# Aedelon/MASt3R-SLAM

Measured on AMD Instinct MI355X. Metric: keyframe-pairs/sec (512x512 two-view infer+match+GN), higher is better.
Workload: dtype fp16

## Files before the change

### mast3r-slam_amd/csrc/conv_tail.hip

```cpp
#include "gemm_common.h"

using namespace m3gemm;

namespace {

constexpr int kThreads = 512;
constexpr int TH = 16, TW = 32;
constexpr int HH = TH + 2, HW = TW + 2;
constexpr int kHaloPix = HH * HW;
constexpr int kHaloBytes = kHaloPix * 128;
constexpr int kWStage = 128 * 128;
constexpr int PH = 11, PW = 19;
constexpr int kPatchBytes = (PH * PW * 128 + 1023) / 1024 * 1024;
constexpr int kLdsBytes = kHaloBytes + 2 * kWStage + kPatchBytes;

struct TailArgs {
    const bf16_t *X;
    const bf16_t *Wc;
    const float *bias;
    const bf16_t *W4;
    const float *b4;
    float *pts, *conf;
    bf16_t *Y;
    const bf16_t *R;
    int cout, relu_in;
    const bf16_t *zero16;
    int B, H, W, IH, IW;
    const bf16_t *Wc2, *W42;
    const float *bias2, *b42;
};

enum { EP_PLAIN = 0 , EP_TAIL = 1 , EP_RELU = 2 ,
       EP_ADD = 3  };

template <int DT, bool UPS, int CIN, int EP>
__global__ void __launch_bounds__(kThreads, 2)
k_conv_tail(const TailArgs ain) {
    constexpr bool TAIL = EP == EP_TAIL;
    static_assert(CIN % 64 == 0 && (TAIL ? CIN == 128 : true), "64-channel steps; the fused tail is the 128-channel head.2");
    constexpr int NQ = CIN / 64;
    TailArgs a = ain;
    if (blockIdx.y == 1) {
        a.Wc = ain.Wc2; a.W4 = ain.W42; a.bias = ain.bias2; a.b4 = ain.b42;
        a.X = ain.X + (size_t)ain.B * ain.IH * ain.IW * CIN;
        if (TAIL) {
            a.pts = ain.pts + (size_t)ain.B * ain.H * ain.W * 3;
            a.conf = ain.conf + (size_t)ain.B * ain.H * ain.W;
        } else {
            a.Y = ain.Y + (size_t)ain.B * ain.H * ain.W * ain.cout;
            if (EP == EP_ADD) a.R = ain.R + (size_t)ain.B * ain.H * ain.W * ain.cout;
        }
    }
    if (!TAIL) {
        const int z = blockIdx.z;
        a.Wc += (size_t)z * 128 * 9 * CIN;
        if (a.bias) a.bias += z * 128;
        a.Y += z * 128;
        if (EP == EP_ADD) a.R += z * 128;
    }
    extern __shared__ __attribute__((aligned(16))) unsigned char lds[];
    unsigned char *halo = lds, *wst = lds + kHaloBytes, *patch = lds + kHaloBytes + 2 * kWStage;
    const int tid = threadIdx.x, lane = tid & 63, wave = tid >> 6;
    const int wp = wave >> 1, wc = wave & 1;
    const int tiles_x = (a.W + TW - 1) / TW, tiles_y = a.H / TH;
    const int nwg = tiles_x * tiles_y * a.B;
    const int bid = xcd_remap(blockIdx.x, nwg);
    const int b = bid / (tiles_x * tiles_y), trem = bid - b * tiles_x * tiles_y;
    const int ty = trem / tiles_x, tx = trem - ty * tiles_x;
    const int oy0 = ty * TH, ox0 = tx * TW;
    const bf16_t *img = a.X + (size_t)b * a.IH * a.IW * CIN;

    auto stage_w = [&](int tap, int half, int buf) {
        unsigned char *base = wst + buf * kWStage;
#pragma unroll
        for (int i = 0; i < 2; ++i) {
            const int slot = i * kThreads + tid;
            const int row = slot >> 3, cp = slot & 7;
            const int c = half * 8 + (cp ^ ((row >> 1) & 7));
            glds16(a.Wc + ((size_t)row * 9 + tap) * CIN + c * 8, base + i * (kThreads * 16) + wave * 1024);
        }
    };
    const float sy = UPS && a.H > 1 ? (float)(a.IH - 1) / (float)(a.H - 1) : 0.f;
    const float sx = UPS && a.W > 1 ? (float)(a.IW - 1) / (float)(a.W - 1) : 0.f;
    const int py0 = (int)((float)max(oy0 - 1, 0) * sy), px0 = (int)((float)max(ox0 - 1, 0) * sx);
    auto stage_patch = [&](int half) {
        for (int wi = wave; wi < (PH * PW * 8 + 63) / 64; wi += kThreads / 64) {
            int slot = wi * 64 + lane;
            slot = slot < PH * PW * 8 ? slot : PH * PW * 8 - 1;
            const int pp = slot >> 3, c = slot & 7;
            const int y = min(py0 + pp / PW, a.IH - 1), x = min(px0 + pp % PW, a.IW - 1);
            glds16(img + ((size_t)y * a.IW + x) * CIN + (half * 8 + c) * 8, patch + wi * 1024);
        }
    };
    auto stage_halo_direct = [&](int half) {
        for (int wi = wave; wi < (kHaloPix * 8 + 63) / 64; wi += kThreads / 64) {
            int slot = wi * 64 + lane;
            const bool live = slot < kHaloPix * 8;
            slot = live ? slot : kHaloPix * 8 - 1;
            const int pix = slot >> 3, cp = slot & 7;
            const int hy = pix / HW, hx = pix - hy * HW;
            const int iy = oy0 + hy - 1, ix = ox0 + hx - 1;
            const int c = half * 8 + (cp ^ ((hx >> 1) & 7));
            const bool in = iy >= 0 && iy < a.H && ix >= 0 && ix < a.W;
            const void *src = in ? (const void *)(img + ((size_t)iy * a.IW + ix) * CIN + c * 8) : (const void *)a.zero16;
            if (wi * 64 + 64 <= kHaloPix * 8) glds16(src, halo + wi * 1024);
            else if (live) *reinterpret_cast<uint4 *>(halo + (size_t)slot * 16) = *reinterpret_cast<const uint4 *>(src);
        }
    };
    auto blend_halo = [&]() {
        for (int slot = tid; slot < kHaloPix * 8; slot += kThreads) {
            const int pix = slot >> 3, cp = slot & 7;
            const int hy = pix / HW, hx = pix - hy * HW;
            const int iy = oy0 + hy - 1, ix = ox0 + hx - 1;
            const int c = cp ^ ((hx >> 1) & 7);
            uint4 o = make_uint4(0u, 0u, 0u, 0u);
            if (iy >= 0 && iy < a.H && ix >= 0 && ix < a.W) {
                const float fy = iy * sy, fx = ix * sx;
                int y0 = (int)fy, x0 = (int)fx;
                y0 = min(y0, a.IH - 1); x0 = min(x0, a.IW - 1);
                const int y1 = min(y0 + 1, a.IH - 1), x1 = min(x0 + 1, a.IW - 1);
                const float wy = fy - (float)y0, wx = fx - (float)x0;
                const unsigned char *p = patch + c * 16;
                union U { uint4 q; unsigned w[4]; } q00, q01, q10, q11, r;
                q00.q = *reinterpret_cast<const uint4 *>(p + ((y0 - py0) * PW + (x0 - px0)) * 128);
                q01.q = *reinterpret_cast<const uint4 *>(p + ((y0 - py0) * PW + (x1 - px0)) * 128);
                q10.q = *reinterpret_cast<const uint4 *>(p + ((y1 - py0) * PW + (x0 - px0)) * 128);
                q11.q = *reinterpret_cast<const uint4 *>(p + ((y1 - py0) * PW + (x1 - px0)) * 128);
#pragma unroll
                for (int k = 0; k < 4; ++k) {
                    const float tl = lo16<DT>(q00.w[k]) * (1.f - wx) + lo16<DT>(q01.w[k]) * wx;
                    const float bl = lo16<DT>(q10.w[k]) * (1.f - wx) + lo16<DT>(q11.w[k]) * wx;
                    const float th = hi16<DT>(q00.w[k]) * (1.f - wx) + hi16<DT>(q01.w[k]) * wx;
                    const float bh = hi16<DT>(q10.w[k]) * (1.f - wx) + hi16<DT>(q11.w[k]) * wx;
                    r.w[k] = pack16<DT>(tl * (1.f - wy) + bl * wy, th * (1.f - wy) + bh * wy);
                }
                o = r.q;
            }
            *reinterpret_cast<uint4 *>(halo + (size_t)slot * 16) = o;
        }
    };

    f32x4 acc[8][4];
#pragma unroll
    for (int i = 0; i < 8; ++i)
#pragma unroll
        for (int j = 0; j < 4; ++j) acc[i][j] = f32x4{0.f, 0.f, 0.f, 0.f};
    const int frow = lane & 15, fch = lane >> 4;
    int w_off[4];
#pragma unroll
    for (int j = 0; j < 4; ++j) {
        const int r = wc * 64 + j * 16 + frow;
        w_off[j] = r * 128 + ((fch ^ ((r >> 1) & 7)) << 4);
    }

    const int group = wave >> 2;
    bf16x8 af[8], wf[4];
    const int pix_of_row = (int)((0x3D9F2A40E6C851B7ULL >> (4 * frow)) & 15);
    auto col_offset = [&](int hx) { return hx * 128 + ((fch ^ ((hx >> 1) & 7)) << 4); };
    auto read_frags = [&](int g, int tap, int ks) {
        const int ky = tap / 3, kx = tap - ky * 3;
        const unsigned char *wsrc = wst + (g & 1) * kWStage;
        const int flip = ks << 6;
        const int c0 = col_offset(pix_of_row + kx) ^ flip;
        const int c1 = col_offset(16 + pix_of_row + kx) ^ flip;
        const unsigned char *rowp = halo + (wp * 4 + ky) * (HW * 128);
#pragma unroll
        for (int j = 0; j < 4; ++j) wf[j] = *reinterpret_cast<const bf16x8 *>(wsrc + (w_off[j] ^ flip));
#pragma unroll
        for (int i = 0; i < 8; ++i)
            af[i] = *reinterpret_cast<const bf16x8 *>(rowp + (i >> 1) * (HW * 128) + ((i & 1) ? c1 : c0));
        if (!TAIL && a.relu_in) {
#pragma unroll
            for (int i = 0; i < 8; ++i) af[i] = relu_frag(af[i]);
        }
    };
    auto mfma_all = [&]() {
        __builtin_amdgcn_s_setprio(1);
#pragma unroll
        for (int i = 0; i < 8; ++i)
#pragma unroll
            for (int j = 0; j < 4; ++j) acc[i][j] = mfma16<DT>(wf[j], af[i], acc[i][j]);
        __builtin_amdgcn_s_setprio(0);
    };
    auto phase_end = [&]() {
        __builtin_amdgcn_sched_barrier(0);
        __builtin_amdgcn_s_barrier();
        __builtin_amdgcn_sched_barrier(0);
    };
    auto phase_end_wait = [&]() {
        __builtin_amdgcn_sched_barrier(0);
        asm volatile("s_waitcnt vmcnt(0)" ::: "memory");
        __builtin_amdgcn_s_barrier();
        __builtin_amdgcn_sched_barrier(0);
    };
    auto prefetch_w = [&](int g) { if (g + 1 < 9 * NQ) stage_w((g + 1) % 9, (g + 1) / 9, (g + 1) & 1); };
    auto run_half = [&](int half) {
        if (group == 0) {
#pragma unroll 1
            for (int tap = 0; tap < 9; ++tap) {
                const int g = half * 9 + tap;
                read_frags(g, tap, 0);
                prefetch_w(g);
                asm volatile("s_waitcnt lgkmcnt(0)" ::: "memory");
                phase_end();
                mfma_all();
                phase_end();
                read_frags(g, tap, 1);
                asm volatile("s_waitcnt lgkmcnt(0)" ::: "memory");
                phase_end();
                mfma_all();
                phase_end_wait();
            }
            phase_end();
        } else {
#pragma unroll 1
            for (int tap = 0; tap < 9; ++tap) {
                const int g = half * 9 + tap;
                if (tap > 0) mfma_all();
                phase_end();
                read_frags(g, tap, 0);
                prefetch_w(g);
                asm volatile("s_waitcnt lgkmcnt(0)" ::: "memory");
                phase_end();
                mfma_all();
                phase_end();
                read_frags(g, tap, 1);
                asm volatile("s_waitcnt lgkmcnt(0)" ::: "memory");
                phase_end_wait();
            }
            mfma_all();
            phase_end();
        }
    };

    stage_w(0, 0, 0);
    if (UPS) stage_patch(0); else stage_halo_direct(0);
    asm volatile("s_waitcnt vmcnt(0)" ::: "memory");
    lds_barrier();
#pragma unroll 1
    for (int q = 0; q < NQ; ++q) {
        if (UPS) {
            blend_halo();
            lds_barrier();
            if (q + 1 < NQ) stage_patch(q + 1);
        } else if (q > 0) {
            stage_halo_direct(q);
            asm volatile("s_waitcnt vmcnt(0)" ::: "memory");
            lds_barrier();
        }
        run_half(q);
    }

    if constexpr (EP == EP_ADD) {
        const int r = lane & 15, gq = lane >> 4;
        constexpr int RS = 272;
        unsigned char *wl = halo + wave * (32 * RS);
        float4 bj[4];
#pragma unroll
        for (int j = 0; j < 4; ++j)
            bj[j] = a.bias ? *reinterpret_cast<const float4 *>(a.bias + wc * 64 + j * 16 + gq * 4) : make_float4(0.f, 0.f, 0.f, 0.f);
        auto pix = [&](int pass, int rl, int &oy, int &ox) {
            const int i = pass * 2 + (rl >> 4);
            oy = oy0 + wp * 4 + (i >> 1);
            ox = ox0 + (i & 1) * 16 + (int)((0x3D9F2A40E6C851B7ULL >> (4 * (rl & 15))) & 15);
        };
        uint4 q[2][4];
        auto load_resid = [&](int pass, uint4 (&dst)[4]) {
#pragma unroll
            for (int it = 0; it < 4; ++it) {
                const int c = it * 64 + lane, rl = c >> 3, ch = c & 7;
                int oy, ox;
                pix(pass, rl, oy, ox);
                ox = ox < a.W ? ox : a.W - 1;
                dst[it] = *reinterpret_cast<const uint4 *>(a.R + (((size_t)b * a.H + oy) * a.W + ox) * a.cout + wc * 64 + ch * 8);
            }
        };
        load_resid(0, q[0]);
#pragma unroll
        for (int pass = 0; pass < 4; ++pass) {
            if (pass + 1 < 4) load_resid(pass + 1, q[(pass + 1) & 1]);
#pragma unroll
            for (int ii = 0; ii < 2; ++ii)
#pragma unroll
                for (int j = 0; j < 4; ++j) {
                    const f32x4 v = acc[pass * 2 + ii][j];
                    *reinterpret_cast<float4 *>(wl + (ii * 16 + r) * RS + ((j * 4 + gq) << 4)) =
                        make_float4(v[0] + bj[j].x, v[1] + bj[j].y, v[2] + bj[j].z, v[3] + bj[j].w);
                }
            asm volatile("s_waitcnt lgkmcnt(0)" ::: "memory");
#pragma unroll
            for (int it = 0; it < 4; ++it) {
                const int c = it * 64 + lane, rl = c >> 3, ch = c & 7;
                const float4 f0 = *reinterpret_cast<const float4 *>(wl + rl * RS + ch * 32);
                const float4 f1 = *reinterpret_cast<const float4 *>(wl + rl * RS + ch * 32 + 16);
                const uint4 u = q[pass & 1][it];
                uint4 o;
                o.x = pack16<DT>(f0.x + lo16<DT>(u.x), f0.y + hi16<DT>(u.x));
                o.y = pack16<DT>(f0.z + lo16<DT>(u.y), f0.w + hi16<DT>(u.y));
                o.z = pack16<DT>(f1.x + lo16<DT>(u.z), f1.y + hi16<DT>(u.z));
                o.w = pack16<DT>(f1.z + lo16<DT>(u.w), f1.w + hi16<DT>(u.w));
                int oy, ox;
                pix(pass, rl, oy, ox);
                if (ox < a.W)
                    *reinterpret_cast<uint4 *>(a.Y + (((size_t)b * a.H + oy) * a.W + ox) * a.cout + wc * 64 + ch * 8) = o;
            }
            asm volatile("" ::: "memory");
        }
    } else if constexpr (!TAIL) {
        const int r = lane & 15, gq = lane >> 4;
        unsigned char *wl = halo + wave * 8192;
        float4 bj[4];
#pragma unroll
        for (int j = 0; j < 4; ++j)
            bj[j] = a.bias ? *reinterpret_cast<const float4 *>(a.bias + wc * 64 + j * 16 + gq * 4) : make_float4(0.f, 0.f, 0.f, 0.f);
#pragma unroll
        for (int pass = 0; pass < 2; ++pass) {
#pragma unroll
            for (int ii = 0; ii < 4; ++ii)
#pragma unroll
                for (int j = 0; j < 4; ++j) {
                    f32x4 v = acc[pass * 4 + ii][j];
                    v[0] += bj[j].x; v[1] += bj[j].y; v[2] += bj[j].z; v[3] += bj[j].w;
                    if (EP == EP_RELU) {
#pragma unroll
                        for (int e = 0; e < 4; ++e) v[e] = v[e] > 0.f ? v[e] : 0.f;
                    }
                    uint2 pk;
                    pk.x = pack16<DT>(v[0], v[1]); pk.y = pack16<DT>(v[2], v[3]);
                    *reinterpret_cast<uint2 *>(wl + (ii * 16 + r) * 128 + (((j * 2 + (gq >> 1)) ^ ((r >> 1) & 7)) << 4) + (((gq ^ r) & 1) << 3)) = pk;
                }
            asm volatile("s_waitcnt lgkmcnt(0)" ::: "memory");
#pragma unroll
            for (int it = 0; it < 8; ++it) {
                const int c = it * 64 + lane, rl = c >> 3, ch = c & 7;
                uint4 v = *reinterpret_cast<const uint4 *>(wl + rl * 128 + ((ch ^ ((rl >> 1) & 7)) << 4));
                if (rl & 1) v = uint4{v.z, v.w, v.x, v.y};
                const int i = pass * 4 + (rl >> 4);
                const int oy = oy0 + wp * 4 + (i >> 1);
                const int ox = ox0 + (i & 1) * 16 + (int)((0x3D9F2A40E6C851B7ULL >> (4 * (rl & 15))) & 15);
                if (ox < a.W)
                    *reinterpret_cast<uint4 *>(a.Y + (((size_t)b * a.H + oy) * a.W + ox) * a.cout + wc * 64 + ch * 8) = v;
            }
            asm volatile("" ::: "memory");
        }
    } else {
        const int r = lane & 15, gq = lane >> 4;
        float part[8][4];
    #pragma unroll
        for (int i = 0; i < 8; ++i)
    #pragma unroll
            for (int o = 0; o < 4; ++o) part[i][o] = 0.f;
    #pragma unroll
        for (int j = 0; j < 4; ++j) {
            const int n = wc * 64 + j * 16 + gq * 4;
            const float4 bq = a.bias ? *reinterpret_cast<const float4 *>(a.bias + n) : make_float4(0.f, 0.f, 0.f, 0.f);
            float w4[4][4];
    #pragma unroll
            for (int o = 0; o < 4; ++o) {
                const uint2 q = *reinterpret_cast<const uint2 *>(a.W4 + (size_t)o * 128 + n);
                w4[o][0] = lo16<DT>(q.x); w4[o][1] = hi16<DT>(q.x); w4[o][2] = lo16<DT>(q.y); w4[o][3] = hi16<DT>(q.y);
            }
    #pragma unroll
            for (int i = 0; i < 8; ++i) {
                const f32x4 v = acc[i][j];
                const float h[4] = {fmaxf(v[0] + bq.x, 0.f), fmaxf(v[1] + bq.y, 0.f), fmaxf(v[2] + bq.z, 0.f), fmaxf(v[3] + bq.w, 0.f)};
    #pragma unroll
                for (int o = 0; o < 4; ++o)
                    part[i][o] += (h[0] * w4[o][0] + h[1] * w4[o][1]) + (h[2] * w4[o][2] + h[3] * w4[o][3]);
            }
        }
    #pragma unroll
        for (int i = 0; i < 8; ++i)
    #pragma unroll
            for (int o = 0; o < 4; ++o) {
                float v = part[i][o];
                v += __shfl_xor(v, 16, 64);
                v += __shfl_xor(v, 32, 64);
                part[i][o] = v;
            }
        float *red = reinterpret_cast<float *>(wst);
        if (gq == 0) {
    #pragma unroll
            for (int i = 0; i < 8; ++i)
                *reinterpret_cast<float4 *>(red + (((wp * 2 + wc) * 8 + i) * 16 + r) * 4) = make_float4(part[i][0], part[i][1], part[i][2], part[i][3]);
        }
        __syncthreads();
        {
            const int i = 4 * wc + gq;
            const float4 p0 = *reinterpret_cast<const float4 *>(red + (((wp * 2 + 0) * 8 + i) * 16 + r) * 4);
            const float4 p1 = *reinterpret_cast<const float4 *>(red + (((wp * 2 + 1) * 8 + i) * 16 + r) * 4);
            const int oy = oy0 + wp * 4 + (i >> 1), ox = ox0 + (i & 1) * 16 + pix_of_row;
            if (ox < a.W) {
                const float x = p0.x + p1.x + a.b4[0], y = p0.y + p1.y + a.b4[1];
                const float z = p0.z + p1.z + a.b4[2], c = p0.w + p1.w + a.b4[3];
                const float d = sqrtf(x * x + y * y + z * z);
                const float sc = expm1f(d) / fmaxf(d, 1e-8f);
                const size_t m = ((size_t)b * a.H + oy) * a.W + ox;
                a.pts[3 * m + 0] = x * sc; a.pts[3 * m + 1] = y * sc; a.pts[3 * m + 2] = z * sc;
                a.conf[m] = 1.0f + expf(c);
            }
        }
    }
}

}

extern "C" {

static int dpt_tail_launch(const void *X, const void *Wc, const float *bias, const void *W4, const float *b4,
                           const void *Wc2, const float *bias2, const void *W42, const float *b42, float *pts,
                           float *conf, void *Y, const void *R, const void *zero16, int B, int H, int W, int cin, int cout,
                           int ep, int relu_in, int upsample, int dtype, void *stream) {
    const int groups = Wc2 ? 2 : 1;
    const bool tail = ep == EP_TAIL;
    M3_REQUIRE(X && Wc && zero16 && B > 0 && H > 0 && W > 0 && H % 16 == 0 && W % 16 == 0);
    M3_REQUIRE(tail ? (W4 && b4 && pts && conf && cin == 128 && !Y)
                    : (Y && (cin == 128 || cin == 256) && (cout == 128 || cout == 256) && (ep == EP_PLAIN || ep == EP_RELU || ep == EP_ADD)));
    M3_REQUIRE((ep == EP_ADD) == (R != nullptr) && (!upsample || ep == EP_PLAIN || tail));
    M3_REQUIRE(groups == 1 || ((!tail || (W42 && b42)) && (bias == nullptr) == (bias2 == nullptr)));
    M3_REQUIRE((dtype == DT_BF16 || dtype == DT_F16) && (!upsample || (H % 2 == 0 && W % 2 == 0)));
    M3_REQUIRE((int64_t)groups * B * H * W < (1ll << 31));
    M3_REQUIRE(reinterpret_cast<uintptr_t>(X) % 16 == 0 && reinterpret_cast<uintptr_t>(Wc) % 16 == 0 &&
               reinterpret_cast<uintptr_t>(Y) % 16 == 0 && reinterpret_cast<uintptr_t>(R) % 16 == 0);
    TailArgs a;
    a.Wc2 = (const bf16_t *)Wc2; a.W42 = (const bf16_t *)W42; a.bias2 = bias2; a.b42 = b42;
    a.X = (const bf16_t *)X; a.Wc = (const bf16_t *)Wc; a.bias = bias; a.W4 = (const bf16_t *)W4; a.b4 = b4;
    a.pts = pts; a.conf = conf; a.Y = (bf16_t *)Y; a.R = (const bf16_t *)R; a.cout = tail ? 128 : cout; a.relu_in = relu_in;
    a.zero16 = (const bf16_t *)zero16; a.B = B; a.H = H; a.W = W;
    a.IH = upsample ? H / 2 : H; a.IW = upsample ? W / 2 : W;
    const dim3 grid((unsigned)((H / TH) * ((W + TW - 1) / TW) * B), groups, tail ? 1 : cout / 128), blk(kThreads);
    hipStream_t st = (hipStream_t)stream;
#define M3_TAIL(DTV, UP, CI, EPV)                                                                                \
    do {                                                                                                         \
        static M3AttrOnce once;                                                                                  \
        int dev__;                                                                                               \
        if (m3_attr_need(once, &dev__)) {                                                                        \
            M3_CHECK_HIP(hipFuncSetAttribute(reinterpret_cast<const void *>(&k_conv_tail<DTV, UP, CI, EPV>),     \
                                             hipFuncAttributeMaxDynamicSharedMemorySize, kLdsBytes), "m3_dpt_tail/attr"); \
            m3_attr_done(once, dev__);                                                                           \
        }                                                                                                        \
        hipLaunchKernelGGL((k_conv_tail<DTV, UP, CI, EPV>), grid, blk, kLdsBytes, st, a);                        \
    } while (0)
#define M3_TAIL_DT(UP, CI, EPV) do { if (dtype == DT_F16) M3_TAIL(DT_F16, UP, CI, EPV); else M3_TAIL(DT_BF16, UP, CI, EPV); } while (0)
    if (tail) { if (upsample) M3_TAIL_DT(true, 128, EP_TAIL); else M3_TAIL_DT(false, 128, EP_TAIL); }
    else if (ep == EP_PLAIN && cin == 128) { if (upsample) M3_TAIL_DT(true, 128, EP_PLAIN); else M3_TAIL_DT(false, 128, EP_PLAIN); }
    else if (ep == EP_PLAIN) { if (upsample) M3_TAIL_DT(true, 256, EP_PLAIN); else M3_TAIL_DT(false, 256, EP_PLAIN); }
    else if (ep == EP_RELU) { if (cin == 128) M3_TAIL_DT(false, 128, EP_RELU); else M3_TAIL_DT(false, 256, EP_RELU); }
    else { if (cin == 128) M3_TAIL_DT(false, 128, EP_ADD); else M3_TAIL_DT(false, 256, EP_ADD); }
#undef M3_TAIL_DT
#undef M3_TAIL
    M3_CHECK_LAUNCH("m3_dpt_tail");
    return M3_OK;
}

int m3_dpt_tail_grouped2_dt(const void *X, const void *Wc0, const void *Wc1, const float *bias0, const float *bias1,
                            const void *W40, const void *W41, const float *b40, const float *b41, float *pts,
                            float *conf, const void *zero16, int B, int H, int W, int upsample, int dtype, void *stream) {
    M3_REQUIRE(pts && conf && (Wc1 == nullptr) == (W41 == nullptr));
    if (!Wc1) bias1 = b41 = nullptr;
    return dpt_tail_launch(X, Wc0, bias0, W40, b40, Wc1, bias1, W41, b41, pts, conf, nullptr, nullptr, zero16, B, H, W, 128, 128,
                           EP_TAIL, 0, upsample, dtype, stream);
}

int m3_conv3x3_up_direct_grouped2_dt(const void *X, const void *Wc0, const void *Wc1, const float *bias0, const float *bias1,
                                     void *Y, const void *zero16, int B, int H, int W, int Cin, int upsample, int dtype,
                                     void *stream) {
    M3_REQUIRE(Y != nullptr);
    return dpt_tail_launch(X, Wc0, bias0, nullptr, nullptr, Wc1, Wc1 ? bias1 : nullptr, nullptr, nullptr, nullptr, nullptr, Y,
                           nullptr, zero16, B, H, W, Cin, 128, EP_PLAIN, 0, upsample, dtype, stream);
}

int m3_conv3x3_direct_grouped2_dt(const void *X, const void *W0, const void *W1, const float *bias0, const float *bias1,
                                  void *Y, const void *R, const void *zero16, int B, int H, int W, int Cin, int Cout,
                                  int epilogue, int dtype, void *stream) {
    const int relu_in = (epilogue & 0x100) ? 1 : 0;
    const int e = epilogue & 0xff;
    M3_REQUIRE(Y != nullptr && (e == M3_EPI_BF16 || e == M3_EPI_BF16_RELU || e == M3_EPI_BF16_ADD));
    const int ep = e == M3_EPI_BF16 ? EP_PLAIN : (e == M3_EPI_BF16_RELU ? EP_RELU : EP_ADD);
    return dpt_tail_launch(X, W0, bias0, nullptr, nullptr, W1, bias1, nullptr, nullptr, nullptr, nullptr, Y, R, zero16, B, H, W,
                           Cin, Cout, ep, relu_in, 0, dtype, stream);
}

}
```

Baseline: 287.5.

## Precompute halo slot addresses, table-driven separable bilinear blend, permlane reductions in tail

Halo staging now computes per-lane source pixel offsets and chunk swizzles once, outside the channel-half loop, instead of redoing the divisions and bounds checks on every pass. The upsampling blend uses a small LDS table of per-row and per-column interpolation indices and weights, and walks rows in groups so horizontal interpolations are reused across neighbouring output rows. The tail epilogue's cross-lane sums use permlane16/32 swap builtins instead of shuffles, and its dot products use explicit FMAs. This adds LDS usage and register pressure, and relies on the gfx950 permlane swap intrinsics.

```diff
diff --git a/mast3r-slam_amd/csrc/conv_tail.hip b/mast3r-slam_amd/csrc/conv_tail.hip
--- a/mast3r-slam_amd/csrc/conv_tail.hip
+++ b/mast3r-slam_amd/csrc/conv_tail.hip
@@ -12,7 +12,12 @@
 constexpr int kWStage = 128 * 128;
 constexpr int PH = 11, PW = 19;
 constexpr int kPatchBytes = (PH * PW * 128 + 1023) / 1024 * 1024;
-constexpr int kLdsBytes = kHaloBytes + 2 * kWStage + kPatchBytes;
+constexpr int kBlendTabBytes = 512;
+constexpr int kLdsBytes = kHaloBytes + 2 * kWStage + kPatchBytes + kBlendTabBytes;
+constexpr int kHaloWI = (kHaloPix * 8 + 63) / 64;
+constexpr int kSlotsPerLane = (kHaloWI + kThreads / 64 - 1) / (kThreads / 64);
+constexpr int kRowGroup = 6, kColItems = HW * 8;
+constexpr int kGroupWI = (kColItems + 63) / 64;
 
 struct TailArgs {
     const bf16_t *X;
@@ -32,6 +37,15 @@
 
 enum { EP_PLAIN = 0 , EP_TAIL = 1 , EP_RELU = 2 ,
        EP_ADD = 3  };
+
+__device__ __forceinline__ float sum_xor16(float v) {
+    const auto r = __builtin_amdgcn_permlane16_swap(__float_as_uint(v), __float_as_uint(v), false, false);
+    return __uint_as_float(r[0]) + __uint_as_float(r[1]);
+}
+__device__ __forceinline__ float sum_xor32(float v) {
+    const auto r = __builtin_amdgcn_permlane32_swap(__float_as_uint(v), __float_as_uint(v), false, false);
+    return __uint_as_float(r[0]) + __uint_as_float(r[1]);
+}
 
 template <int DT, bool UPS, int CIN, int EP>
 __global__ void __launch_bounds__(kThreads, 2)
@@ -92,51 +106,102 @@
             glds16(img + ((size_t)y * a.IW + x) * CIN + (half * 8 + c) * 8, patch + wi * 1024);
         }
     };
+    const int wave_u = __builtin_amdgcn_readfirstlane(wave);
+    int spix[kSlotsPerLane];
+    unsigned schunk = 0;
+#pragma unroll
+    for (int k = 0; k < kSlotsPerLane; ++k) {
+        const int slot = min((wave_u + k * (kThreads / 64)) * 64 + lane, kHaloPix * 8 - 1);
+        const int pix = slot >> 3, cp = slot & 7;
+        const int hy = pix / HW, hx = pix - hy * HW;
+        const int iy = oy0 + hy - 1, ix = ox0 + hx - 1;
+        const bool in = iy >= 0 && iy < a.H && ix >= 0 && ix < a.W;
+        spix[k] = in ? iy * a.IW + ix : -1;
+        schunk |= (unsigned)(cp ^ ((hx >> 1) & 7)) << (3 * k);
+    }
     auto stage_halo_direct = [&](int half) {
-        for (int wi = wave; wi < (kHaloPix * 8 + 63) / 64; wi += kThreads / 64) {
-            int slot = wi * 64 + lane;
-            const bool live = slot < kHaloPix * 8;
-            slot = live ? slot : kHaloPix * 8 - 1;
-            const int pix = slot >> 3, cp = slot & 7;
-            const int hy = pix / HW, hx = pix - hy * HW;
-            const int iy = oy0 + hy - 1, ix = ox0 + hx - 1;
-            const int c = half * 8 + (cp ^ ((hx >> 1) & 7));
-            const bool in = iy >= 0 && iy < a.H && ix >= 0 && ix < a.W;
-            const void *src = in ? (const void *)(img + ((size_t)iy * a.IW + ix) * CIN + c * 8) : (const void *)a.zero16;
+#pragma unroll
+        for (int k = 0; k < kSlotsPerLane; ++k) {
+            const int wi = wave_u + k * (kThreads / 64);
+            if (wi >= kHaloWI) break;
+            const int c = half * 8 + (int)((schunk >> (3 * k)) & 7);
+            const void *src = spix[k] >= 0 ? (const void *)(img + (size_t)spix[k] * CIN + c * 8) : (const void *)a.zero16;
             if (wi * 64 + 64 <= kHaloPix * 8) glds16(src, halo + wi * 1024);
-            else if (live) *reinterpret_cast<uint4 *>(halo + (size_t)slot * 16) = *reinterpret_cast<const uint4 *>(src);
-        }
+            else if (wi * 64 + lane < kHaloPix * 8)
+                *reinterpret_cast<uint4 *>(halo + (size_t)(wi * 64 + lane) * 16) = *reinterpret_cast<const uint4 *>(src);
+        }
+    };
+    uint2 *btab = reinterpret_cast<uint2 *>(lds + kHaloBytes + 2 * kWStage + kPatchBytes);
+    auto blend_entry = [](int i, int n, int ni, float s, int p0) {
+        const float f = i * s;
+        int i0 = (int)f;
+        i0 = min(i0, ni - 1);
+        const int i1 = min(i0 + 1, ni - 1);
+        const float w = f - (float)i0;
+        return i >= 0 && i < n ? make_uint2(__float_as_uint(w), (unsigned)((i0 - p0) | ((i1 - p0) << 8) | (1 << 16))) : make_uint2(0u, 0u);
+    };
+    auto fill_blend_table = [&]() {
+        if (tid < HH) btab[tid] = blend_entry(oy0 + tid - 1, a.H, a.IH, sy, py0);
+        else if (tid < HH + HW) btab[tid] = blend_entry(ox0 + (tid - HH) - 1, a.W, a.IW, sx, px0);
     };
     auto blend_halo = [&]() {
-        for (int slot = tid; slot < kHaloPix * 8; slot += kThreads) {
-            const int pix = slot >> 3, cp = slot & 7;
-            const int hy = pix / HW, hx = pix - hy * HW;
-            const int iy = oy0 + hy - 1, ix = ox0 + hx - 1;
-            const int c = cp ^ ((hx >> 1) & 7);
-            uint4 o = make_uint4(0u, 0u, 0u, 0u);
-            if (iy >= 0 && iy < a.H && ix >= 0 && ix < a.W) {
-                const float fy = iy * sy, fx = ix * sx;
-                int y0 = (int)fy, x0 = (int)fx;
-                y0 = min(y0, a.IH - 1); x0 = min(x0, a.IW - 1);
-                const int y1 = min(y0 + 1, a.IH - 1), x1 = min(x0 + 1, a.IW - 1);
-                const float wy = fy - (float)y0, wx = fx - (float)x0;
-                const unsigned char *p = patch + c * 16;
-                union U { uint4 q; unsigned w[4]; } q00, q01, q10, q11, r;
-                q00.q = *reinterpret_cast<const uint4 *>(p + ((y0 - py0) * PW + (x0 - px0)) * 128);
-                q01.q = *reinterpret_cast<const uint4 *>(p + ((y0 - py0) * PW + (x1 - px0)) * 128);
-                q10.q = *reinterpret_cast<const uint4 *>(p + ((y1 - py0) * PW + (x0 - px0)) * 128);
-                q11.q = *reinterpret_cast<const uint4 *>(p + ((y1 - py0) * PW + (x1 - px0)) * 128);
+#pragma unroll 1
+        for (int wi = wave_u; wi < 3 * kGroupWI; wi += kThreads / 64) {
+            const int grp = wi / kGroupWI, item = (wi - grp * kGroupWI) * 64 + lane;
+            if (item >= kColItems) continue;
+            const int hx = item >> 3, cp = item & 7;
+            const uint2 xe = btab[HH + hx];
+            const float wx = __uint_as_float(xe.x), owx = 1.f - wx;
+            const bool xin = (xe.y >> 16) != 0;
+            const unsigned char *p0 = patch + ((cp ^ ((hx >> 1) & 7)) << 4);
+            const unsigned char *p1 = p0 + ((xe.y >> 8) & 0xff) * 128;
+            p0 += (xe.y & 0xff) * 128;
+            unsigned char *dst = halo + (grp * kRowGroup * HW * 8 + item) * 16;
+            union U { uint4 q; unsigned w[4]; };
+            auto hrow = [&](float (&t)[8], int yr) {
+                U qa, qb;
+                qa.q = *reinterpret_cast<const uint4 *>(p0 + yr * (PW * 128));
+                qb.q = *reinterpret_cast<const uint4 *>(p1 + yr * (PW * 128));
 #pragma unroll
                 for (int k = 0; k < 4; ++k) {
-                    const float tl = lo16<DT>(q00.w[k]) * (1.f - wx) + lo16<DT>(q01.w[k]) * wx;
-                    const float bl = lo16<DT>(q10.w[k]) * (1.f - wx) + lo16<DT>(q11.w[k]) * wx;
-                    const float th = hi16<DT>(q00.w[k]) * (1.f - wx) + hi16<DT>(q01.w[k]) * wx;
-                    const float bh = hi16<DT>(q10.w[k]) * (1.f - wx) + hi16<DT>(q11.w[k]) * wx;
-                    r.w[k] = pack16<DT>(tl * (1.f - wy) + bl * wy, th * (1.f - wy) + bh * wy);
+                    t[2 * k] = __builtin_fmaf(lo16<DT>(qb.w[k]), wx, lo16<DT>(qa.w[k]) * owx);
+                    t[2 * k + 1] = __builtin_fmaf(hi16<DT>(qb.w[k]), wx, hi16<DT>(qa.w[k]) * owx);
                 }
-                o = r.q;
-            }
-            *reinterpret_cast<uint4 *>(halo + (size_t)slot * 16) = o;
+            };
+            float ta[8], tb[8];
+            int ha = -1, hb = -1;
+#pragma unroll 1
+            for (int r = 0; r < kRowGroup; ++r) {
+                const uint2 ye = btab[grp * kRowGroup + r];
+                const unsigned yi = __builtin_amdgcn_readfirstlane(ye.y);
+                const float wy = __uint_as_float(__builtin_amdgcn_readfirstlane(ye.x)), owy = 1.f - wy;
+                U o;
+                o.q = make_uint4(0u, 0u, 0u, 0u);
+                if (yi >> 16) {
+                    const int y0 = yi & 0xff, y1 = (yi >> 8) & 0xff;
+                    if (y0 != ha) {
+                        if (y0 == hb) {
+#pragma unroll
+                            for (int k = 0; k < 8; ++k) ta[k] = tb[k];
+                        } else hrow(ta, y0);
+                        ha = y0;
+                    }
+                    if (y1 != hb) {
+                        if (y1 == ha) {
+#pragma unroll
+                            for (int k = 0; k < 8; ++k) tb[k] = ta[k];
+                        } else hrow(tb, y1);
+                        hb = y1;
+                    }
+#pragma unroll
+                    for (int k = 0; k < 4; ++k) {
+                        const unsigned v = pack16<DT>(__builtin_fmaf(tb[2 * k], wy, ta[2 * k] * owy),
+                                                      __builtin_fmaf(tb[2 * k + 1], wy, ta[2 * k + 1] * owy));
+                        o.w[k] = xin ? v : 0u;
+                    }
+                }
+                *reinterpret_cast<uint4 *>(dst + r * (HW * 128)) = o.q;
+            }
         }
     };
 
@@ -234,7 +299,7 @@
     };
 
     stage_w(0, 0, 0);
-    if (UPS) stage_patch(0); else stage_halo_direct(0);
+    if (UPS) { stage_patch(0); fill_blend_table(); } else stage_halo_direct(0);
     asm volatile("s_waitcnt vmcnt(0)" ::: "memory");
     lds_barrier();
 #pragma unroll 1
@@ -366,17 +431,15 @@
                 const float h[4] = {fmaxf(v[0] + bq.x, 0.f), fmaxf(v[1] + bq.y, 0.f), fmaxf(v[2] + bq.z, 0.f), fmaxf(v[3] + bq.w, 0.f)};
     #pragma unroll
                 for (int o = 0; o < 4; ++o)
-                    part[i][o] += (h[0] * w4[o][0] + h[1] * w4[o][1]) + (h[2] * w4[o][2] + h[3] * w4[o][3]);
+                    part[i][o] += (o & 1) ? __builtin_fmaf(h[0], w4[o][0], h[1] * w4[o][1]) + __builtin_fmaf(h[2], w4[o][2], h[3] * w4[o][3])
+                                          : __builtin_fmaf(h[1], w4[o][1], h[0] * w4[o][0]) + __builtin_fmaf(h[3], w4[o][3], h[2] * w4[o][2]);
             }
         }
     #pragma unroll
         for (int i = 0; i < 8; ++i)
     #pragma unroll
             for (int o = 0; o < 4; ++o) {
-                float v = part[i][o];
-                v += __shfl_xor(v, 16, 64);
-                v += __shfl_xor(v, 32, 64);
-                part[i][o] = v;
+                part[i][o] = sum_xor32(sum_xor16(part[i][o]));
             }
         float *red = reinterpret_cast<float *>(wst);
         if (gq == 0) {
```

Result: no change. 289.5, median of 6 (+0.7%).
